# Borx25/CPU-Raytracing-experiments

Hardware: AMD Instinct MI355X
Metric: Mray/s (primary+bounce) (higher is better)
Workload: dtype f32; 1 GPU; cfg4: 4096x4096 px, S(100000) spheres + SAH BVH, MIS, Policy.max_bounces=9 (primary+8 bounces), 5 buckets, 64 accumulations/step; fixed image, tile rows split over the GPUs; image=4096x4096, spheres=100000, max_bounces=9, buckets=5, parallelism=single GPU, batches_in_flight=1, accumulations_per_batch=63, accumulations_per_batch_limit=63

## Files before the change

cpu-raytracing-experiments_amd/__init__.py:

```python
from __future__ import annotations

import ctypes as C
import os
import subprocess

import numpy as np

from . import distributed as distributed
from . import hdr as hdr
from . import scene as scene
from .scene import MATERIAL, NODE, SPHERE, Camera, Scene

_HERE = os.path.dirname(os.path.abspath(__file__))
CSRC = os.path.join(_HERE, "csrc")
LIB_PATH = os.path.join(CSRC, "libmirt.so")

MIRT_OK, MIRT_NOT_READY = 0, 1
MIRT_NOT_CONVERGED = 2
NOISE_BINS = 2048
AOV_DEPTH, AOV_NORMAL, AOV_ALBEDO = 0, 1, 2
AOV_PLANES = 7
KERNEL_CLASSES = ("raygen", "trace", "shade", "shadow", "resolve")


# ... 44 lines not shown

def load_library():
    global _lib
    if _lib is not None:
        return _lib
    if not os.path.exists(LIB_PATH):
        raise MirtError(f"{LIB_PATH} not built — run __graft_entry__.build() (hipcc --offload-arch=gfx950); there is no CPU fallback")
    lib = C.CDLL(LIB_PATH)
    P, u32, i32, f, vp = C.c_void_p, C.c_uint32, C.c_int, C.c_float, C.c_void_p
    sigs = {
        "mirt_create": [i32, C.POINTER(P)],
        "mirt_destroy": [P],
        "mirt_bvh_build": [vp, u32, vp, C.POINTER(u32), vp],
        "mirt_light_list": [vp, u32, vp, u32, vp, C.POINTER(u32)],
        "mirt_set_scene": [P, vp, vp, u32, vp, u32, vp, u32, vp, u32, vp, vp, u32, u32],
        "mirt_set_camera": [P, vp, vp, f, f, f, f],
        "mirt_set_lens": [P, f, f], "mirt_get_lens": [P, C.POINTER(f), C.POINTER(f)],
        "mirt_pick_focus": [P, u32, u32, C.POINTER(f), C.POINTER(f)],
        "mirt_set_policy": [P, C.POINTER(Policy)],
        "mirt_get_policy": [P, C.POINTER(Policy)],
        "mirt_set_gloss_decay": [P, vp, u32],
        "mirt_set_stream_order": [P, u32], "mirt_get_stream_order": [P, C.POINTER(u32)],
        "mirt_resize": [P, u32, u32],
        "mirt_set_tile_range": [P, u32, u32], "mirt_set_tile_rows": [P, u32, u32],
        "mirt_reset": [P],
        "mirt_accumulate": [P, u32],
        "mirt_accumulate_async": [P, u32],
        "mirt_synchronize": [P],
        "mirt_get_accumulations": [P, C.POINTER(u32)],
        "mirt_accumulator_floats": [P, C.POINTER(C.c_size_t)],
        "mirt_read_accumulator": [P, vp],
        "mirt_accumulator_device": [P, C.POINTER(vp), C.POINTER(C.c_size_t)],
        "mirt_load_accumulator": [P, vp, i32, u32],
        "mirt_render": [P, vp],
        "mirt_set_aov": [P, u32], "mirt_get_aov": [P, C.POINTER(u32)],
        "mirt_aov_floats": [P, C.POINTER(C.c_size_t)],
        "mirt_read_aov": [P, vp],
        "mirt_aov_device": [P, C.POINTER(vp), C.POINTER(C.c_size_t)],
        "mirt_load_aov": [P, vp, i32],
        "mirt_render_aov": [P, i32, vp],
        "mirt_noise": [P, f, vp, vp, vp, C.POINTER(NoiseStats)],
        "mirt_noise_quantile": [vp, C.c_double, C.POINTER(f)],
        "mirt_accumulate_until": [P, C.POINTER(StopRule), C.POINTER(NoiseStats), C.POINTER(u32)],
        "mirt_get_counters": [P, C.POINTER(Counters)],
        "mirt_get_kernel_times": [P, C.POINTER(KernelTimes), i32],
        "mirt_get_stream": [P, C.POINTER(vp)],
        "mirt_debug_raygen": [P, u32, vp, vp],
        "mirt_debug_trace_closest": [P, C.c_size_t, vp, vp, vp, vp],
        "mirt_debug_trace_shadow": [P, C.c_size_t, vp, vp, vp, vp],
        "mirt_debug_math": [P, i32, C.c_size_t, vp, vp],
        "mirt_debug_info": [P, vp],
        "mirt_debug_tree": [P, vp, C.c_size_t, vp],
        "mirt_debug_primary_lists": [P, vp],
        "mirt_debug_allow_half_boxes": [P, i32],
    }
    G = C.c_void_p
    sigs.update({
        "mirt_group_create": [vp, i32, C.POINTER(G)],
        "mirt_group_destroy": [G],
        "mirt_group_size": [G, C.POINTER(i32)],
        "mirt_group_member": [G, i32, C.POINTER(P)],
        "mirt_group_set_scene": [G, vp, vp, u32, vp, u32, vp, u32, vp, u32, vp, vp, u32, u32],
        "mirt_group_set_camera": [G, vp, vp, f, f, f, f],
        "mirt_group_set_lens": [G, f, f],
        "mirt_group_pick_focus": [G, u32, u32, C.POINTER(f), C.POINTER(f)],
        "mirt_group_set_policy": [G, C.POINTER(Policy)],
        "mirt_group_set_gloss_decay": [G, vp, u32],
        "mirt_group_set_stream_order": [G, u32],
        "mirt_group_resize": [G, u32, u32],
        "mirt_group_reset": [G],
        "mirt_group_accumulate": [G, u32],
        "mirt_group_accumulate_async": [G, u32],
        "mirt_group_synchronize": [G],
        "mirt_group_get_accumulations": [G, C.POINTER(u32)],
        "mirt_group_get_counters": [G, C.POINTER(Counters)],
        "mirt_group_gather": [G],
        "mirt_group_last_gather_ms": [G, C.POINTER(C.c_double)],
        "mirt_group_accumulator_floats": [G, C.POINTER(C.c_size_t)],
        "mirt_group_read_accumulator": [G, vp],
        "mirt_group_render": [G, vp],
        "mirt_group_set_aov": [G, u32],
        "mirt_group_aov_floats": [G, C.POINTER(C.c_size_t)],
        "mirt_group_read_aov": [G, vp],
        "mirt_group_render_aov": [G, i32, vp],
        "mirt_group_noise": [G, f, vp, vp, vp, C.POINTER(NoiseStats)],
        "mirt_group_accumulate_until": [G, C.POINTER(StopRule), C.POINTER(NoiseStats), C.POINTER(u32)],
        "mirt_group_rccl_selftest": [i32, C.c_size_t],
    })
    for name, argtypes in sigs.items():
        fn = getattr(lib, name)
        fn.argtypes = argtypes
        fn.restype = C.c_int
    lib.mirt_last_error.argtypes = [P]
    lib.mirt_last_error.restype = C.c_char_p
    lib.mirt_group_last_error.argtypes = [P]
    lib.mirt_group_last_error.restype = C.c_char_p
    lib._declared = tuple(sigs) + ("mirt_last_error", "mirt_group_last_error")
    _lib = lib
    return lib


def _ptr(a: np.ndarray):
    return a.ctypes.data_as(C.c_void_p)


def bvh_build(geometry: np.ndarray):
# ... 265 lines not shown
        ptr = C.c_void_p(src) if is_device else _ptr(np.ascontiguousarray(src, dtype=np.float32))
        self._check(self._lib.mirt_load_aov(self._ctx, ptr, int(is_device)))

    def render_aov(self, which: int, out: np.ndarray = None):
        img = _aov_image(self.height, self.width, which, out)
        rc = self._check(self._lib.mirt_render_aov(self._ctx, int(which), _ptr(img)))
        return img if rc == MIRT_OK else None

    noise_quantile = staticmethod(noise_quantile)

    def _local_tiles(self) -> int:
        n = C.c_size_t(0)
        self._check(self._lib.mirt_accumulator_floats(self._ctx, C.byref(n)))
        return n.value // (self.policy.buckets * 768)

    def noise(self, floor: float = 0.0, want_map: bool = False, map_out: np.ndarray = None):
        return _noise(self._lib.mirt_noise, self._check, self._ctx, self.height, self.width, self._local_tiles(), floor, want_map, map_out)

    def accumulate_until(self, target: float, quantile: float = 0.95, floor: float = 0.0, check_every: int = None, max_accumulations: int = 1000):
        return _accumulate_until(self._lib.mirt_accumulate_until, self._check, self._ctx, self.policy.buckets, target, quantile, floor, check_every, max_accumulations)

    def counters(self) -> dict:
        c = Counters()
        self._check(self._lib.mirt_get_counters(self._ctx, C.byref(c)))
        return c.as_dict()

    def kernel_times(self, reset: bool = True) -> dict:
        t = KernelTimes()
        self._check(self._lib.mirt_get_kernel_times(self._ctx, C.byref(t), int(reset)))
        return {k: {"ms": t.ms[i], "launches": int(t.launches[i])} for i, k in enumerate(KERNEL_CLASSES)}

    def debug_info(self) -> dict:
        out = (C.c_uint32 * 8)()
        self._check(self._lib.mirt_debug_info(self._ctx, out))
        keys = ("records", "lds_records", "lds_spheres", "depth", "half_boxes", "trace_lds_bytes", "trace_workgroups_per_cu", "cus")
        d = dict(zip(keys, [int(v) for v in out]))
        d["wide"] = (d["half_boxes"] >> 1) & 1
        d["half_boxes"] &= 1
        return d

    def debug_tree(self):
        info = (C.c_uint32 * 4)()
        self._check(self._lib.mirt_debug_tree(self._ctx, None, 0, info))
        n, rec_bytes = int(info[0]), int(info[1])
        words = np.zeros((n, rec_bytes // 4), dtype=np.uint32)
        self._check(self._lib.mirt_debug_tree(self._ctx, _ptr(words), words.nbytes, info))
        return words, dict(zip(("records", "record_bytes", "layout", "depth"), [int(v) for v in info]))

    def debug_primary_lists(self) -> list:
        out = (C.c_uint32 * 10)()
        self._check(self._lib.mirt_debug_primary_lists(self._ctx, out))
        return [int(v) for v in out]

    def stream_handle(self) -> int:
        p = C.c_void_p()
        self._check(self._lib.mirt_get_stream(self._ctx, C.byref(p)))
        return p.value

    def debug_raygen(self, accumulations: int):
        n = (self.width // 16) * (self.height // 16) * 256
        p = np.empty((3, n), dtype=np.float32)
        d = np.empty((3, n), dtype=np.float32)
        self._check(self._lib.mirt_debug_raygen(self._ctx, accumulations, _ptr(p), _ptr(d)))
        return p, d

    def debug_trace_closest(self, p: np.ndarray, d: np.ndarray):
        p = np.ascontiguousarray(p, dtype=np.float32); d = np.ascontiguousarray(d, dtype=np.float32)
        n = p.shape[1]
        tfar = np.empty(n, dtype=np.float32); prim = np.empty(n, dtype=np.int32)
        self._check(self._lib.mirt_debug_trace_closest(self._ctx, n, _ptr(p), _ptr(d), _ptr(tfar), _ptr(prim)))
        return tfar, prim

    def debug_trace_shadow(self, p: np.ndarray, d: np.ndarray, tfar: np.ndarray):
        p = np.ascontiguousarray(p, dtype=np.float32); d = np.ascontiguousarray(d, dtype=np.float32)
        tfar = np.ascontiguousarray(tfar, dtype=np.float32)
        n = p.shape[1]
        occ = np.empty(n, dtype=np.uint8)
        self._check(self._lib.mirt_debug_trace_shadow(self._ctx, n, _ptr(p), _ptr(d), _ptr(tfar), _ptr(occ)))
        return occ

    def debug_math(self, fn: int, inputs: np.ndarray, n_out: int) -> np.ndarray:
        inputs = np.ascontiguousarray(inputs, dtype=np.float32)
        n = inputs.shape[-1]
        out = np.empty((n_out, n), dtype=np.float32)
        self._check(self._lib.mirt_debug_math(self._ctx, fn, n, _ptr(inputs), _ptr(out)))
        return out


class GroupRenderer:

    def __init__(self, scene: Scene, devices=(0,), max_bounces: int = 16, buckets: int = 5, mis: bool = True, use_bvh: bool = True,
                 count_traffic: bool = False, max_batch: int = 0, streams: int = 0, reference_tree: bool = False, gpu_build: bool = False,
                 brdf: int = 0, gloss_decay=None, exact_stream_order: bool = False, aov: bool = False, lens: bool = False):
        self._lib = load_library()
        self._g = C.c_void_p()
        self._lens_follows_camera = bool(lens)
        dev = (C.c_int * len(devices))(*devices)
        rc = self._lib.mirt_group_create(dev, len(devices), C.byref(self._g))
        if rc != MIRT_OK:
            raise MirtError(f"mirt_group_create failed ({rc}): {self._lib.mirt_group_last_error(None).decode()}")
        self.scene, self.devices = scene, tuple(devices)
        self.width = self.height = 0
        self.framebuffer = None
        self.policy = Policy(max_bounces, buckets, int(mis), int(use_bvh), int(count_traffic), 0, max_batch, int(reference_tree), int(streams), int(gpu_build), 0,
                             int(brdf))
        self._check(self._lib.mirt_group_set_policy(self._g, C.byref(self.policy)))
# ... 159 lines not shown
```

cpu-raytracing-experiments_amd/csrc/kernels.hpp:

```cpp
#pragma once
#include <hip/hip_runtime.h>
#include <stdint.h>
#include "device_math.hpp"

namespace mirt {

constexpr uint32_t kBlock = 256;
constexpr uint32_t kShadeBlock = 512;
constexpr uint32_t kTraceBlock = 1024;
constexpr uint32_t kLdsStack = 16;
constexpr uint32_t kLdsStackWide = 12;
constexpr uint32_t kLeafBit = 0x80000000u;
constexpr uint32_t kTileSize = 256;
constexpr uint32_t kTileRoot = 16;
constexpr uint32_t kStack = 64;
constexpr uint32_t kDestAccum = 0x80000000u;

struct SceneDev {
	const float4* recs;
	const float4* spheres;
	const int32_t* prim_mat;
	const float4* light_sphere;
	const float4* light_emit;
	const float4* mat_albedo;
	const float4* mat_emission;
	const float4* hdri;
	uint32_t n_spheres, n_recs, n_mat, n_lights;
	uint32_t lds_recs;
	uint32_t lds_spheres;
	uint32_t half_boxes;
	uint32_t wide;
	uint32_t chunk_max;
	uint32_t leaf_batch;
	uint32_t refill_idle;
	uint32_t stack16;
	float ambient[3];
	int32_t hdri_w, hdri_h;
	float hdri_fw, hdri_fh;
	uint32_t has_ambient;
	uint32_t use_bvh;
};

struct StreamBuf {
	float *px, *py, *pz, *dx, *dy, *dz;
	float *tr, *tg, *tb;
	uint32_t* path;
};
struct ShadowBuf {
	float *px, *py, *pz;
	float *dx, *dy, *dz, *tfar;
	float *sr, *sg, *sb;
	float *er, *eg, *eb;
	uint32_t* dest;
};
struct FrameParams {
	CameraParams cam;
// ... 752 lines not shown
	};
	auto store_result = [&](uint32_t pix, const Trav& t, bool) {
		const bool over = static_cast<uint32_t>(t.prim) > kCandMax;
		cand[pix] = over ? kCandOverflow : static_cast<uint32_t>(t.prim);
		const unsigned long long m = __ballot(over);
		if (over) {
			const uint32_t leader = static_cast<uint32_t>(__ffsll(static_cast<long long>(m))) - 1u;
			uint32_t first = 0;
			if (lane_id() == leader) first = atomicAdd(ov_count, static_cast<uint32_t>(__popcll(m)));
			first = __builtin_amdgcn_readlane(first, leader);
			if (ov_pix) ov_pix[first + mask_rank(m)] = pix;
		}
	};
	trace_queue<kCollect, COUNT>(sc, tl, Queue{ nullptr, 0u }, n, work, unused, c_nodes, c_spheres, load_ray, store_result, Collect{ cand, rho, n });
	if (COUNT) { wave_sum(c_nodes, &ctr->nodes); wave_sum(c_spheres, &ctr->spheres); }
}
constexpr uint32_t kCandRegs = 3;
template <bool COUNT>
__global__ __launch_bounds__(kBlock) void k_primary_hits(SceneDev sc, FrameParams fp, const uint32_t* __restrict__ cand, HitRec* __restrict__ hit_out, DevCounters* ctr) {
	if (blockIdx.x == 0 && threadIdx.x == 0 && fp.n_pix) atomicAdd(&ctr->rays, static_cast<unsigned long long>(fp.n_pix) * fp.batch_n);
	uint32_t c_spheres = 0;
	const float ox = fp.cam.pos[0], oy = fp.cam.pos[1], oz = fp.cam.pos[2];
	for (uint32_t pix = blockIdx.x * kBlock + threadIdx.x; pix < fp.n_pix; pix += gridDim.x * kBlock) {
		const uint32_t cnt = cand[pix];
		if (cnt == kCandOverflow) continue;
		uint32_t tile; int32_t x, y;
		pixel_xy(fp, pix, tile, x, y);
		const uint32_t seed = (tile * kTileSize + (pix & 255u)) * (fp.max_bounces * 2u + 1u);
		float4 s[kCandRegs]; int32_t id[kCandRegs];
		for (uint32_t k = 0; k < kCandRegs; k++) {
			id[k] = k < cnt ? static_cast<int32_t>(cand[static_cast<size_t>(k + 1u) * fp.n_pix + pix]) : -1;
			s[k] = sc.spheres[id[k] < 0 ? 0 : id[k]];
		}
		for (uint32_t slot = 0; slot < fp.batch_n; slot++) {
			uint32_t rng = hash_2d(fp.acc_base + slot + 1u, seed);
			const float s0 = rand_unit_float(rng);
			const float s1 = rand_unit_float(rng);
			const f3 d = camera_ray_dir(fp.cam, x, y, s0, s1);
			float tfar = MIRT_FLT_MAX; int32_t prim = -1;
			for (uint32_t k = 0; k < kCandRegs; k++) if (id[k] >= 0) sphere_closest_tie(s[k], id[k], ox, oy, oz, d.x, d.y, d.z, tfar, prim);
			for (uint32_t k = kCandRegs; k < kCandMax; k++) {
				if (__ballot(k < cnt) == 0ull) break;
				if (k < cnt) {
					const uint32_t j = cand[static_cast<size_t>(k + 1u) * fp.n_pix + pix];
					sphere_closest_tie(sc.spheres[j], static_cast<int32_t>(j), ox, oy, oz, d.x, d.y, d.z, tfar, prim);
				}
			}
			if (COUNT) c_spheres += cnt;
			const size_t i = static_cast<size_t>(slot) * fp.n_pix + pix;
			hit_out[i] = HitRec{ tfar, prim };
		}
	}
	if (COUNT) wave_sum(c_spheres, &ctr->spheres);
}

constexpr uint32_t kAovPlanes = 7;
constexpr float kAovMissDepth = 1e4f;
template <bool LENS = false>
__global__ __launch_bounds__(kBlock) void k_first_hit_aov(SceneDev sc, FrameParams fp, const HitRec* __restrict__ hit_in, const float4* __restrict__ mat_colour, float* __restrict__ aov, LensParams lens) {
	f3 O{ fp.cam.pos[0], fp.cam.pos[1], fp.cam.pos[2] };
	for (uint32_t pix = blockIdx.x * kBlock + threadIdx.x; pix < fp.n_pix; pix += gridDim.x * kBlock) {
		uint32_t tile; int32_t x, y;
		pixel_xy(fp, pix, tile, x, y);
		const uint32_t seed = (tile * kTileSize + (pix & 255u)) * (fp.max_bounces * 2u + 1u);
		float* w = aov + static_cast<size_t>(pix >> 8) * (kAovPlanes * kTileSize) + (pix & 255u);
		float sum[kAovPlanes];
		for (uint32_t k = 0; k < kAovPlanes; k++) sum[k] = w[k * kTileSize];
		int32_t cached = -1;
		float4 hs = make_float4(0.0f, 0.0f, 0.0f, 0.0f), colour = hs;
		for (uint32_t slot = 0; slot < fp.batch_n; slot++) {
			uint32_t rng = hash_2d(fp.acc_base + slot + 1u, seed);
			const float s0 = rand_unit_float(rng);
			const float s1 = rand_unit_float(rng);
			f3 D = camera_ray_dir(fp.cam, x, y, s0, s1);
			if (LENS) lens_ray(fp.cam, lens, D, fp.acc_base + slot + 1u, seed, fp.max_bounces, O, D);
			const HitRec h = hit_in[static_cast<size_t>(slot) * fp.n_pix + pix];
			if (h.prim < 0) { sum[0] += kAovMissDepth; continue; }
			if (h.prim != cached) { hs = sc.spheres[h.prim]; colour = mat_colour[sc.prim_mat[h.prim]]; cached = h.prim; }
			const float depth = h.tfar;
			const f3 hit{ O.x + D.x * depth, O.y + D.y * depth, O.z + D.z * depth };
			f3 N = normalize3(f3{ hit.x - hs.x, hit.y - hs.y, hit.z - hs.z });
			if (dot3(N, D) >= 0.0f) N = f3{ -N.x, -N.y, -N.z };
			sum[0] += depth;
			sum[1] += N.x; sum[2] += N.y; sum[3] += N.z;
			sum[4] += colour.x; sum[5] += colour.y; sum[6] += colour.z;
		}
		for (uint32_t k = 0; k < kAovPlanes; k++) w[k * kTileSize] = sum[k];
	}
}
constexpr int kAovDepth = 0, kAovNormal = 1, kAovAlbedo = 2;
__global__ __launch_bounds__(kBlock) void k_resolve_aov(const float* __restrict__ aov, float* __restrict__ out, uint32_t n_pix, uint32_t first_tile, uint32_t run_tiles,
                                                        uint32_t stride_tiles, uint32_t h_tiles, uint32_t width, int which, float accumulations) {
	for (uint32_t pix = blockIdx.x * kBlock + threadIdx.x; pix < n_pix; pix += gridDim.x * kBlock) {
		const float* src = aov + static_cast<size_t>(pix >> 8) * (kAovPlanes * kTileSize) + (pix & 255u);
		const uint32_t tile = global_tile(first_tile, run_tiles, stride_tiles, pix >> 8), ID = pix & 255u;
		const uint32_t x = kTileRoot * (tile % h_tiles) + (ID & 15u);
		const uint32_t y = kTileRoot * (tile / h_tiles) + (ID >> 4);
		const size_t at = static_cast<size_t>(y) * width + x;
		if (which == kAovDepth) { out[at] = src[0] / accumulations; continue; }
		const uint32_t first = which == kAovNormal ? 1u : 4u;
		f3 v{ src[first * kTileSize], src[(first + 1u) * kTileSize], src[(first + 2u) * kTileSize] };
		if (which == kAovNormal) v = dot3(v, v) == 0.0f ? f3{ 0.0f, 0.0f, 0.0f } : normalize3(v);
		else v = { v.x / accumulations, v.y / accumulations, v.z / accumulations };
		out[at * 3u] = v.x; out[at * 3u + 1u] = v.y; out[at * 3u + 2u] = v.z;
	}
}
// ... 680 lines not shown
```

cpu-raytracing-experiments_amd/csrc/mirt_capi.hip:

```cpp
#include "../../include/mirt.h"
#include "kernels.hpp"
#include "bvh_layout.hpp"
#include "bvh_build.hpp"
#include "lbvh_build.hpp"
#include "noise_host.hpp"

#include <hip/hip_runtime.h>
#include <algorithm>
#include <cstdarg>
#include <cstdint>
#include <cstdio>
#include <cstdlib>
#include <cstring>
#include <string>
#include <vector>

using namespace mirt;

namespace {

thread_local std::string g_create_error;

struct DeviceBuffer {
	void* ptr = nullptr;
// ... 330 lines not shown
float bundle_half_angle(const mirt_ctx* c) { return (0.7072f / std::fabs(c->camera.z)) * 1.01f + 1e-4f; }

void update_lens_axes(mirt_ctx* c) {
	const f3 r = camera_axis(c->camera.orient, f3{ 1.0f, 0.0f, 0.0f }), u = camera_axis(c->camera.orient, f3{ 0.0f, 1.0f, 0.0f }), f = camera_axis(c->camera.orient, f3{ 0.0f, 0.0f, -1.0f });
	c->lens.right[0] = r.x; c->lens.right[1] = r.y; c->lens.right[2] = r.z;
	c->lens.up[0] = u.x; c->lens.up[1] = u.y; c->lens.up[2] = u.z;
	c->lens.fwd[0] = f.x; c->lens.fwd[1] = f.y; c->lens.fwd[2] = f.z;
}
bool lens_on(const mirt_ctx* c) { return c->lens.aperture > 0.0f; }

FrameParams frame_params(const mirt_ctx* c, uint32_t acc_base, uint32_t batch_n) {
	FrameParams fp{};
	fp.cam = c->camera;
	fp.h_tiles = c->h_tiles;
	fp.first_tile = c->first_tile;
	fp.run_tiles = c->run_tiles ? c->run_tiles : 1u;
	fp.stride_tiles = c->stride_tiles;
	fp.n_pix = c->n_tiles * kTileSize;
	fp.pix_bits = pix_bits_of(c); fp.pix_mask = (1u << fp.pix_bits) - 1u;
	fp.acc_base = acc_base;
	fp.batch_n = batch_n;
	fp.max_bounces = c->policy.max_bounces;
	fp.buckets = c->policy.buckets;
	fp.n_lights = c->scene.n_lights;
	fp.mis = (c->policy.mis && c->scene.n_lights > 0) ? 1u : 0u;
	fp.first_groups = 1;
	fp.inv_n_pix = fp.n_pix ? 1.0f / static_cast<float>(fp.n_pix) : 0.0f;
	fp.inv_h_tiles = fp.h_tiles ? 1.0f / static_cast<float>(fp.h_tiles) : 0.0f;
	fp.inv_run_tiles = 1.0f / static_cast<float>(fp.run_tiles);
	return fp;
}

SceneDev trace_scene(const mirt_ctx* c) {
	SceneDev sc = c->scene;
	sc.use_bvh = c->policy.use_bvh;
	sc.chunk_max = c->tune_chunk; sc.leaf_batch = c->tune_leaf_batch; sc.refill_idle = c->tune_refill_idle;
	return sc;
}

const decltype(&k_trace<true, kPrimaryNone>) kTrace[2][3] = {
	{ k_trace<true, kPrimaryNone>, k_trace<true, kPrimaryAll>, k_trace<true, kPrimaryList> },
	{ k_trace<false, kPrimaryNone>, k_trace<false, kPrimaryAll>, k_trace<false, kPrimaryList> } };
const decltype(&k_trace_fat<true, kPrimaryNone>) kTraceFat[2][3] = {
	{ k_trace_fat<true, kPrimaryNone>, k_trace_fat<true, kPrimaryAll>, k_trace_fat<true, kPrimaryList> },
	{ k_trace_fat<false, kPrimaryNone>, k_trace_fat<false, kPrimaryAll>, k_trace_fat<false, kPrimaryList> } };
const decltype(&k_primary_cand<true>) kPrimaryCand[2] = { k_primary_cand<true>, k_primary_cand<false> };
const decltype(&k_primary_hits<true>) kPrimaryHits[2] = { k_primary_hits<true>, k_primary_hits<false> };
const decltype(&k_shade<false, false>) kShade[2][2] = { { k_shade<false, false>, k_shade<false, true> }, { k_shade<true, false>, k_shade<true, true> } };
const decltype(&k_tile_stream<false>) kTileStream[2] = { k_tile_stream<false>, k_tile_stream<true> };
static_assert(kPrimaryNone == 0 && kPrimaryAll == 1 && kPrimaryList == 2, "kTrace / kTraceFat are indexed by PRIMARY");
const decltype(&k_trace<true, kPrimaryNone>) kTraceLens[2] = { k_trace<true, kPrimaryAll, true>, k_trace<false, kPrimaryAll, true> };
const decltype(&k_trace_fat<true, kPrimaryNone>) kTraceFatLens[2] = { k_trace_fat<true, kPrimaryAll, true>, k_trace_fat<false, kPrimaryAll, true> };
const decltype(&k_shade<false, false>) kShadeLens[2] = { k_shade<true, false, true>, k_shade<true, true, true> };

struct TraceLaunch {
	StreamBuf in; HitRec* hit;
	Queue closest_queue; uint32_t* closest_work;
	ShadowBuf sh; ShadowSink sink;
	Queue shadow_queue; uint32_t* shadow_work;
	FatList fat_closest, fat_shadow;
	const uint32_t* listed_pixels;
	DevCounters* ctr;
};
void launch_trace(const mirt_ctx* c, hipStream_t st, const SceneDev& sc, const FrameParams& fp, uint64_t n_rays, bool count, int primary, const TraceLaunch& t, bool lens = false) {
	hipLaunchKernelGGL(lens ? kTraceLens[!count] : kTrace[!count][primary], dim3(trace_grid(c, n_rays)), dim3(kTraceBlock), trace_lds(c), st, sc, fp, t.in, t.hit, t.closest_queue, t.closest_work,
	                   t.sh, t.sink, t.shadow_queue, t.shadow_work, t.fat_closest, t.fat_shadow, t.ctr, c->lens);
	const uint32_t fat_grid = sc.n_spheres > 4096 ? static_cast<uint32_t>(c->n_cu) * 2u : 64u;
	if (sc.use_bvh) hipLaunchKernelGGL(lens ? kTraceFatLens[!count] : kTraceFat[!count][primary], dim3(fat_grid), dim3(1024), 0, st, sc, fp, t.in, t.hit, t.fat_closest, t.sh, t.sink, t.fat_shadow, t.ctr, t.listed_pixels, c->lens);
}

int launch_tile_stream(mirt_ctx* c, hipStream_t st, const SceneDev& sc, const FrameParams& fp, uint32_t batch_n, float* contrib, DevCounters* ctr, bool count) {
	if (!c->gloss_decay_dev_valid) {
		HIP_TRY(c, sync_all(c));
		HIP_TRY(c, c->gloss_decay_dev.ensure(std::max<size_t>(c->gloss_decay.size(), 1) * sizeof(float)));
		if (!c->gloss_decay.empty()) HIP_TRY(c, hipMemcpy(c->gloss_decay_dev.ptr, c->gloss_decay.data(), c->gloss_decay.size() * sizeof(float), hipMemcpyHostToDevice));
		c->gloss_decay_dev_valid = true;
	}
	Bracket t(c, MIRT_K_TRACE, st);
	hipLaunchKernelGGL(kTileStream[c->policy.brdf != 0], dim3(c->n_tiles * batch_n), dim3(kTileSize), 0, st, sc, fp, contrib, ctr, c->mat_ggx.as<float4>(),
	                   c->gloss_decay_dev.as<float>(), static_cast<uint32_t>(c->gloss_decay.size()), count ? 1u : 0u);
	return MIRT_OK;
}

int build_primary_lists(mirt_ctx* c, const SceneDev& sc, const FrameParams& fp, bool count) {
	HIP_TRY(c, c->cand.ensure(static_cast<size_t>(fp.n_pix) * kCandStride * sizeof(uint32_t)));
	HIP_TRY(c, c->cand_listed.ensure(static_cast<size_t>(fp.n_pix) * sizeof(uint32_t)));
	HIP_TRY(c, c->cand_words.ensure(CandWords::kWords * sizeof(uint32_t)));
	if (!c->cand_built) HIP_TRY(c, hipEventCreateWithFlags(&c->cand_built, hipEventDisableTiming));
	const CandWords cw{ c->cand_words.as<uint32_t>() };
	HIP_TRY(c, hipMemsetAsync(cw.w, 0, CandWords::kWords * sizeof(uint32_t), c->stream));
	{ Bracket t(c, MIRT_K_TRACE);
	  const FatList none{ cw.unused_fat_count(), nullptr, 0u };
	  hipLaunchKernelGGL(kPrimaryCand[!count], dim3(trace_grid(c, fp.n_pix)), dim3(kTraceBlock), trace_lds(c), c->stream, sc, fp, c->cand.as<uint32_t>(), bundle_half_angle(c),
	                     cw.work(), none, c->counters.as<DevCounters>(), c->cand_listed.as<uint32_t>(), cw.listed_pixels()); }
	HIP_TRY(c, hipGetLastError());
	HIP_TRY(c, hipEventRecord(c->cand_built, c->stream));
	c->cand_gen++;
	c->cand_valid = true;
	return MIRT_OK;
}

int launch_first_hit_aov(mirt_ctx* c, PipeSlot& sl, hipStream_t st, const SceneDev& sc, const FrameParams& fp) {
	const bool pipelined = c->slots.size() > 1;
	if (pipelined) {
		if (!sl.aov_done) HIP_TRY(c, hipEventCreateWithFlags(&sl.aov_done, hipEventDisableTiming));
		if (c->aov_prev && c->aov_prev != sl.aov_done) HIP_TRY(c, hipStreamWaitEvent(st, c->aov_prev, 0));
// ... 1 lines not shown
	{ Bracket t(c, MIRT_K_RESOLVE, st);
	  const uint32_t grid = static_cast<uint32_t>(std::min<uint64_t>((static_cast<uint64_t>(fp.n_pix) + kBlock - 1) / kBlock, static_cast<uint64_t>(c->n_cu) * 64u));
	  hipLaunchKernelGGL(lens_on(c) ? k_first_hit_aov<true> : k_first_hit_aov<false>, dim3(grid), dim3(kBlock), 0, st, sc, fp, sl.hit, c->policy.brdf ? c->mat_ggx.as<float4>() : c->scene.mat_albedo,
	                     c->aov.as<float>(), c->lens); }
	if (pipelined) { HIP_TRY(c, hipEventRecord(sl.aov_done, st)); c->aov_prev = sl.aov_done; }
	return MIRT_OK;
}

int launch_batch(mirt_ctx* c, uint32_t batch_n) {
	FrameParams fp = frame_params(c, c->accumulations, batch_n);
	const uint32_t nb = c->policy.max_bounces;
	const uint64_t total = static_cast<uint64_t>(fp.n_pix) * batch_n;
	if (total == 0) { c->accumulations += batch_n; return MIRT_OK; }
	const bool pipelined = c->slots.size() > 1;
	PipeSlot& sl = c->slots[c->batch_seq % c->slots.size()];
	hipStream_t st = pipelined ? sl.stream : c->stream;
	const BatchCounters bc = batch_counters(c, sl);
	const float qn = c->camera.orient[0] * c->camera.orient[0] + c->camera.orient[1] * c->camera.orient[1] + c->camera.orient[2] * c->camera.orient[2] + c->camera.orient[3] * c->camera.orient[3];
	const bool lens = lens_on(c);
	const bool bundle = c->policy.use_bvh && c->scene.n_recs != 0 && !c->policy.trace_primary_rays && batch_n >= 3 && c->camera.z != 0.0f && std::fabs(qn - 1.0f) < 1e-4f && !c->stream_order && !lens;
	DevCounters* ctr = c->counters.as<DevCounters>();
	const float4* mat_ggx = c->mat_ggx.as<float4>();
	float* contrib = sl.contrib.as<float>();
	uint32_t* fat_lists = sl.fat.as<uint32_t>();
	const SceneDev sc = trace_scene(c);
	const bool count = c->policy.count_traffic != 0;
	const uint32_t sgrid = static_cast<uint32_t>(std::min<uint64_t>((total + kShadeBlock - 1) / kShadeBlock, static_cast<uint64_t>(c->n_cu) * c->tune_shade_wgs));
	{
		const uint64_t n_chunks = (static_cast<uint64_t>(fp.n_pix) + kShadeBlock - 1) / kShadeBlock;
		const uint64_t want = (8ull * sgrid + n_chunks - 1) / n_chunks;
		fp.first_groups = static_cast<uint32_t>(std::min<uint64_t>(std::max<uint64_t>(want, 1), batch_n));
	}

	if (pipelined && sl.in_use) HIP_TRY(c, hipStreamWaitEvent(st, sl.merged, 0));
	if (c->debug_poison_contrib)
		HIP_TRY(c, hipMemsetD32Async(reinterpret_cast<hipDeviceptr_t>(sl.contrib.ptr), 0x7fc0deadu, sl.contrib.bytes / sizeof(float), st));
	HIP_TRY(c, hipMemsetAsync(bc.w, 0, BatchCounters::words(nb) * sizeof(uint32_t), st));
	if (bundle) {
		if (!c->cand_valid || count) { const int r = build_primary_lists(c, sc, fp, count); if (r) return r; }
		if (pipelined && sl.cand_gen != c->cand_gen) { HIP_TRY(c, hipStreamWaitEvent(st, c->cand_built, 0)); sl.cand_gen = c->cand_gen; }
	}
	const CandWords cw{ c->cand_words.as<uint32_t>() };
	if (c->stream_order) {
		const int r = launch_tile_stream(c, st, sc, fp, batch_n, contrib, ctr, count);
		if (r) return r;
	} else {
		for (uint32_t bounce = 0; bounce < nb; bounce++) {
			const StreamBuf& in = sl.stream_buf[bounce & 1u];
			const StreamBuf& out = sl.stream_buf[(bounce & 1u) ^ 1u];
			const bool shadow_pending = fp.mis && bounce > 0;
			const bool lists = bounce == 0 && bundle;
			{ Bracket t(c, MIRT_K_TRACE, st);
			  if (lists) {
			    const uint32_t hgrid = static_cast<uint32_t>(std::min<uint64_t>((static_cast<uint64_t>(fp.n_pix) + kBlock - 1) / kBlock, static_cast<uint64_t>(c->n_cu) * 64u));
			    hipLaunchKernelGGL(kPrimaryHits[!count], dim3(hgrid), dim3(kBlock), 0, st, sc, fp, c->cand.as<uint32_t>(), sl.hit, ctr);
			  }
			  const ShadowSink sink{ in.path, in.px, in.py, in.pz, contrib, batch_n, fp.pix_bits, nullptr };
			  StreamBuf rays = in;
			  if (lists) rays.path = c->cand_listed.as<uint32_t>();
			  const TraceLaunch tl{ rays, sl.hit, lists ? Queue{ cw.listed_pixels(), 0u } : bc.stream_queue(bounce), bc.closest_work(bounce),
			                        sl.shadow_buf, sink, shadow_pending ? bc.shadow_queue(bounce - 1) : bc.empty_queue(), bc.shadow_work(shadow_pending ? bounce - 1 : 0),
			                        bc.fat_closest(bounce, fat_lists), bc.fat_shadow(bounce, fat_lists), lists ? cw.listed_pixels() : nullptr, ctr };
			  launch_trace(c, st, sc, fp, total, count, lists ? kPrimaryList : bounce == 0 ? kPrimaryAll : kPrimaryNone, tl, bounce == 0 && lens); }
			if (bounce == 0 && c->aov_on) { const int r = launch_first_hit_aov(c, sl, st, sc, fp); if (r) return r; }
			{ Bracket t(c, MIRT_K_SHADE, st);
			  const float decay = bounce < c->gloss_decay.size() ? c->gloss_decay[bounce] : 0.0f;
			  hipLaunchKernelGGL(bounce == 0 && lens ? kShadeLens[c->policy.brdf != 0] : kShade[bounce == 0][c->policy.brdf != 0], dim3(sgrid), dim3(kShadeBlock), 0, st, sc, fp, in, sl.hit, out, sl.shadow_buf, bounce,
			                     bc.stream_queue(bounce), bc.stream_queue(bounce + 1), bc.shadow_queue(bounce), contrib, ctr, mat_ggx, decay, c->lens); }
		}
	}
	HIP_TRY(c, hipGetLastError());
	if (pipelined) {
		HIP_TRY(c, hipEventRecord(sl.batch_done, st));
		HIP_TRY(c, hipStreamWaitEvent(c->stream, sl.batch_done, 0));
	}
	{ Bracket t(c, MIRT_K_RESOLVE);
	  hipLaunchKernelGGL(k_merge_contrib, dim3(grid_for(c, static_cast<uint64_t>(c->n_tiles) * (kTileSize / 4u))), dim3(kBlock), 0, c->stream,
	                     c->accumulator.as<float4>(), sl.contrib.as<float4>(), c->n_tiles, c->policy.buckets, batch_n, fp.acc_base); }
	HIP_TRY(c, hipGetLastError());
	if (pipelined) { HIP_TRY(c, hipEventRecord(sl.merged, c->stream)); sl.in_use = true; }
	c->batch_seq++;
	c->accumulations += batch_n;
	if (c->policy.profile && c->pending.size() > 512) harvest(c);
	return MIRT_OK;
}

template <class T>
int upload(mirt_ctx* c, DeviceBuffer& buf, const std::vector<T>& host) {
	HIP_TRY(c, buf.ensure(std::max<size_t>(host.size(), 1) * sizeof(T)));
	if (!host.empty()) HIP_TRY(c, hipMemcpyAsync(buf.ptr, host.data(), host.size() * sizeof(T), hipMemcpyHostToDevice, c->stream));
	return MIRT_OK;
}

int check_ready(mirt_ctx* c) {
	if (!c) return MIRT_ERR_ARG;
	if (!c->have_scene) return fail(c, MIRT_ERR_STATE, "mirt_set_scene has not been called");
	if (!c->have_camera) return fail(c, MIRT_ERR_STATE, "mirt_set_camera has not been called");
	if (c->width == 0 && c->height == 0) return fail(c, MIRT_ERR_STATE, "mirt_resize has not been called");
	return MIRT_OK;
}

int flush_deferred(mirt_ctx* c) {
	if (!c->deferred) return MIRT_OK;
	const uint32_t n = c->deferred;
	c->deferred = 0;
	HIP_TRY(c, hipSetDevice(c->device));
	int r = ensure_streams(c); if (r) return r;
	return launch_batch(c, n);
// ... 699 lines not shown
	if (!c) return MIRT_ERR_ARG;
	if (!c->have_scene) return fail(c, MIRT_ERR_STATE, "mirt_set_scene has not been called");
	if (!p_xyz || !dir_xyz || !tfar_out || !prim_out || n == 0 || n >= (1ull << 31)) return fail(c, MIRT_ERR_ARG, "bad arguments");
	std::vector<HitRec> hits(n);
	const int r = debug_trace(c, "debug_trace_closest", n, p_xyz, dir_xyz, nullptr, hits.data());
	if (r == MIRT_OK) for (size_t i = 0; i < n; i++) { tfar_out[i] = hits[i].tfar; prim_out[i] = hits[i].prim; }
	return r;
}

int mirt_debug_trace_shadow(mirt_ctx* c, size_t n, const float* p_xyz, const float* dir_xyz, const float* tfar, uint8_t* occluded_out) {
	if (!c) return MIRT_ERR_ARG;
	if (!c->have_scene) return fail(c, MIRT_ERR_STATE, "mirt_set_scene has not been called");
	if (!p_xyz || !dir_xyz || !tfar || !occluded_out || n == 0 || n >= (1ull << 31)) return fail(c, MIRT_ERR_ARG, "bad arguments");
	std::vector<uint32_t> occ(n);
	const int r = debug_trace(c, "debug_trace_shadow", n, p_xyz, dir_xyz, tfar, occ.data());
	if (r == MIRT_OK) for (size_t i = 0; i < n; i++) occluded_out[i] = occ[i] ? 1 : 0;
	return r;
}

int mirt_debug_math(mirt_ctx* c, int fn, size_t n, const float* in, float* out) {
	if (!c) return MIRT_ERR_ARG;
	static const int n_in[11] = { 1, 2, 1, 2, 2, 6, 8, 3, 10, 9, 1 }, n_out[11] = { 2, 1, 1, 3, 3, 10, 5, 5, 3, 6, 1 };
	if (fn < 0 || fn > 10 || !in || !out || n == 0 || n >= (1u << 28)) return fail(c, MIRT_ERR_ARG, "bad arguments");
	HIP_TRY(c, hipSetDevice(c->device));
	ScopedBuffer din, dout;
	HIP_TRY(c, din.ensure(n * n_in[fn] * 4)); HIP_TRY(c, dout.ensure(n * n_out[fn] * 4));
	HIP_TRY(c, hipMemcpy(din.ptr, in, n * n_in[fn] * 4, hipMemcpyHostToDevice));
	hipLaunchKernelGGL(k_debug_math, dim3(grid_for(c, n)), dim3(kBlock), 0, c->stream, fn, static_cast<uint32_t>(n), din.as<float>(), dout.as<float>());
	hipError_t e = hipGetLastError();
	if (e == hipSuccess) e = hipStreamSynchronize(c->stream);
	if (e == hipSuccess) e = hipMemcpy(out, dout.ptr, n * n_out[fn] * 4, hipMemcpyDeviceToHost);
	if (e != hipSuccess) return fail(c, MIRT_ERR_HIP, "debug_math: %s", hipGetErrorString(e));
	return MIRT_OK;
}

int mirt_debug_primary_lists(mirt_ctx* c, uint32_t hist[10]) {
	int r = check_ready(c); if (r) return r;
	if (!hist) return fail(c, MIRT_ERR_ARG, "hist is NULL");
	if (!c->policy.use_bvh || c->scene.n_recs == 0 || c->n_tiles == 0) return fail(c, MIRT_ERR_STATE, "needs policy.use_bvh, a tree and at least one tile");
	{ const int fr = flush_deferred(c); if (fr) return fr; }
	HIP_TRY(c, hipSetDevice(c->device));
	if ((r = ensure_streams(c))) return r;
	HIP_TRY(c, sync_all(c));
	const FrameParams fp = frame_params(c, 0, 1);
	if (!c->cand_valid && (r = build_primary_lists(c, trace_scene(c), fp, false))) return r;
	std::vector<uint32_t> host(static_cast<size_t>(fp.n_pix));
	HIP_TRY(c, hipMemcpyAsync(host.data(), c->cand.ptr, host.size() * 4, hipMemcpyDeviceToHost, c->stream));
	HIP_TRY(c, hipStreamSynchronize(c->stream));
	for (int k = 0; k < 10; k++) hist[k] = 0;
	for (size_t p = 0; p < fp.n_pix; p++) { const uint32_t n = host[p]; hist[n == kCandOverflow ? 9 : std::min<uint32_t>(n, 8u)]++; }
	return MIRT_OK;
}

int mirt_debug_info(mirt_ctx* c, uint32_t out[8]) {
	if (!c || !out) return MIRT_ERR_ARG;
	const SceneDev& s = c->scene;
	const LdsPlan p = lds_plan(c);
	out[0] = s.n_recs; out[1] = s.lds_recs; out[2] = s.lds_spheres; out[3] = c->bvh_depth; out[4] = s.half_boxes | (s.wide << 1);
	out[5] = p.launch_bytes; out[6] = p.wgs_per_cu; out[7] = static_cast<uint32_t>(c->n_cu);
	return MIRT_OK;
}
int mirt_debug_tree(mirt_ctx* c, void* dst, size_t capacity_bytes, uint32_t info[4]) {
	if (!c) return MIRT_ERR_ARG;
	if (!info) return fail(c, MIRT_ERR_ARG, "debug_tree: info is NULL");
	if (!c->have_scene) return fail(c, MIRT_ERR_STATE, "mirt_set_scene has not been called");
	const SceneDev& s = c->scene;
	const uint32_t rec_bytes = (s.half_boxes && !s.wide) ? 32u : 64u;
	info[0] = s.n_recs; info[1] = rec_bytes; info[2] = s.wide ? 2u : s.half_boxes ? 1u : 0u; info[3] = c->bvh_depth;
	if (!dst) return MIRT_OK;
	const size_t bytes = static_cast<size_t>(s.n_recs) * rec_bytes;
	if (capacity_bytes < bytes) return fail(c, MIRT_ERR_ARG, "debug_tree: %zu bytes of capacity, the records take %zu", capacity_bytes, bytes);
	if (bytes == 0) return MIRT_OK;
	HIP_TRY(c, hipSetDevice(c->device));
	HIP_TRY(c, hipStreamSynchronize(c->stream));
	HIP_TRY(c, hipMemcpy(dst, s.recs, bytes, hipMemcpyDeviceToHost));
	return MIRT_OK;
}
int mirt_debug_allow_half_boxes(mirt_ctx* c, int allow) { if (!c) return MIRT_ERR_ARG; c->allow_half = allow != 0; return MIRT_OK; }

}
```

include/mirt.h:

```cpp
#ifndef MIRT_H
#define MIRT_H

#include <stddef.h>
#include <stdint.h>

#ifdef __cplusplus
extern "C" {
#endif

#define MIRT_OK              0
#define MIRT_NOT_READY       1
#define MIRT_ERR_ARG        -1
#define MIRT_ERR_HIP        -2
#define MIRT_ERR_STATE      -3
#define MIRT_ERR_NO_DEVICE  -4

#define MIRT_TILE_ROOT     16u
#define MIRT_TILE_SIZE    256u
#define MIRT_MAX_MATERIALS 63u
#define MIRT_MAX_BUCKETS   16u
#define MIRT_BVH_STACK     64u

typedef struct mirt_sphere {
	float   position[3];
// ... 129 lines not shown
	uint32_t max_accumulations;
} mirt_stop_rule;
int mirt_accumulate_until(mirt_ctx* ctx, const mirt_stop_rule* rule, mirt_noise_stats* last, uint32_t* issued);

int mirt_get_counters(mirt_ctx* ctx, mirt_counters* out);
int mirt_get_kernel_times(mirt_ctx* ctx, mirt_kernel_times* out, int reset);
int mirt_get_stream(mirt_ctx* ctx, void** hip_stream);

typedef struct mirt_group mirt_group;
int mirt_group_create(const int* devices, int n, mirt_group** out);
int mirt_group_destroy(mirt_group* group);
const char* mirt_group_last_error(const mirt_group* group);
int mirt_group_size(const mirt_group* group, int* n);
int mirt_group_member(mirt_group* group, int index, mirt_ctx** ctx);
int mirt_group_set_scene(mirt_group* group,
                         const mirt_sphere* geometry, const mirt_sphere* bvh_prims, uint32_t n_spheres,
                         const mirt_bvh_node* nodes, uint32_t n_nodes,
                         const mirt_material* materials, uint32_t n_materials,
                         const int32_t* lights, uint32_t n_lights,
                         const float ambient_color[3], const float* hdri_rgba, uint32_t hdri_w, uint32_t hdri_h);
int mirt_group_set_camera(mirt_group* group, const float pos[3], const float orient_xyzw[4], float half_width, float half_height, float z, float exposure);
int mirt_group_set_lens(mirt_group* group, float aperture_radius, float focus_depth);
int mirt_group_pick_focus(mirt_group* group, uint32_t x, uint32_t y, float* distance, float* depth);
int mirt_group_set_policy(mirt_group* group, const mirt_policy* policy);
int mirt_group_set_gloss_decay(mirt_group* group, const float* decay, uint32_t n);
int mirt_group_set_stream_order(mirt_group* group, uint32_t exact);
int mirt_group_resize(mirt_group* group, uint32_t width, uint32_t height);
int mirt_group_reset(mirt_group* group);
int mirt_group_accumulate(mirt_group* group, uint32_t n_calls);
int mirt_group_accumulate_async(mirt_group* group, uint32_t n_calls);
int mirt_group_synchronize(mirt_group* group);
int mirt_group_get_accumulations(const mirt_group* group, uint32_t* accumulations);
int mirt_group_get_counters(mirt_group* group, mirt_counters* out);
int mirt_group_gather(mirt_group* group);
int mirt_group_last_gather_ms(const mirt_group* group, double* ms);
int mirt_group_accumulator_floats(const mirt_group* group, size_t* n_floats);
int mirt_group_read_accumulator(mirt_group* group, float* host_dst);
int mirt_group_render(mirt_group* group, float* rgba_host);
int mirt_group_set_aov(mirt_group* group, uint32_t on);
int mirt_group_aov_floats(const mirt_group* group, size_t* n_floats);
int mirt_group_read_aov(mirt_group* group, float* host_dst);
int mirt_group_render_aov(mirt_group* group, int which, float* out);
int mirt_group_noise(mirt_group* group, float floor, float* map_out, float* tile_out, uint32_t* hist_out, mirt_noise_stats* stats);
int mirt_group_accumulate_until(mirt_group* group, const mirt_stop_rule* rule, mirt_noise_stats* last, uint32_t* issued);
int mirt_group_rccl_selftest(int device, size_t n_floats);

int mirt_debug_raygen(mirt_ctx* ctx, uint32_t accumulations, float* p_xyz, float* dir_xyz);
int mirt_debug_trace_closest(mirt_ctx* ctx, size_t n, const float* p_xyz, const float* dir_xyz, float* tfar_out, int32_t* primID_out);
int mirt_debug_trace_shadow(mirt_ctx* ctx, size_t n, const float* p_xyz, const float* dir_xyz, const float* tfar, uint8_t* occluded_out);
int mirt_debug_math(mirt_ctx* ctx, int fn, size_t n, const float* in, float* out);
int mirt_debug_info(mirt_ctx* ctx, uint32_t out[8]);
int mirt_debug_tree(mirt_ctx* ctx, void* dst, size_t capacity_bytes, uint32_t info[4]);
int mirt_debug_primary_lists(mirt_ctx* ctx, uint32_t hist[10]);
int mirt_debug_allow_half_boxes(mirt_ctx* ctx, int allow);

#ifdef __cplusplus
}
#endif
#endif
```

Baseline: 9481 Mray/s.

## Add wave-per-pixel-run primary hit kernel with lane-per-sample mapping

Adds a primary-hit kernel in which each wavefront handles a run of 16 pixels in a tile row and each lane handles one accumulation sample. Candidate sphere IDs and sphere data are loaded once per pixel and broadcast across lanes with readlane, and the loads for the next pixels are prefetched. Results pass through LDS and are transposed so the global writes stay coalesced. The aim is to remove redundant per-sample candidate and sphere loads and the divergence of the per-pixel kernel, at the cost of LDS staging, wave barriers, and idle lanes when a group holds fewer than 64 samples. The new path is used only when the batch has at least 32 accumulations. A debug API for reading candidate counts is also added.

```diff
diff --git a/cpu-raytracing-experiments_amd/__init__.py b/cpu-raytracing-experiments_amd/__init__.py
--- a/cpu-raytracing-experiments_amd/__init__.py
+++ b/cpu-raytracing-experiments_amd/__init__.py
@@ -120,6 +120,7 @@
         "mirt_debug_info": [P, vp],
         "mirt_debug_tree": [P, vp, C.c_size_t, vp],
         "mirt_debug_primary_lists": [P, vp],
+        "mirt_debug_primary_counts": [P, vp, C.c_size_t],
         "mirt_debug_allow_half_boxes": [P, i32],
     }
     G = C.c_void_p
@@ -491,6 +492,13 @@
         self._check(self._lib.mirt_debug_primary_lists(self._ctx, out))
         return [int(v) for v in out]
 
+    def debug_primary_counts(self) -> np.ndarray:
+        n = C.c_size_t(0)
+        self._check(self._lib.mirt_accumulator_floats(self._ctx, C.byref(n)))
+        out = np.zeros((n.value // (self.policy.buckets * 768), 256), dtype=np.uint32)
+        self._check(self._lib.mirt_debug_primary_counts(self._ctx, _ptr(out), out.size))
+        return out
+
     def stream_handle(self) -> int:
         p = C.c_void_p()
         self._check(self._lib.mirt_get_stream(self._ctx, C.byref(p)))
diff --git a/cpu-raytracing-experiments_amd/csrc/hits_wave_map.hpp b/cpu-raytracing-experiments_amd/csrc/hits_wave_map.hpp
--- /dev/null
+++ b/cpu-raytracing-experiments_amd/csrc/hits_wave_map.hpp
@@ -0,0 +1,17 @@
+#pragma once
+#include <stdint.h>
+
+namespace mirt {
+
+constexpr uint32_t kWaveHitsMinBatch = 32;
+constexpr uint32_t kWaveHitsRun = 16;
+constexpr uint32_t kWaveHitsPasses = kWaveHitsRun;
+constexpr uint32_t kWaveHitsStage = kWaveHitsRun * 64u;
+
+constexpr uint32_t hits_wave_groups(uint32_t batch_n) { return (batch_n + 63u) >> 6; }
+constexpr uint32_t hits_wave_group_slots(uint32_t batch_n, uint32_t g) { return batch_n - g * 64u < 64u ? batch_n - g * 64u : 64u; }
+constexpr uint32_t hits_wave_stage_index(uint32_t p, uint32_t s) { return p * 64u + (s ^ p); }
+constexpr uint32_t hits_wave_out_pixel(uint32_t lane) { return lane & (kWaveHitsRun - 1u); }
+constexpr uint32_t hits_wave_out_slot(uint32_t lane, uint32_t pass) { return pass * (64u / kWaveHitsRun) + lane / kWaveHitsRun; }
+
+}
diff --git a/cpu-raytracing-experiments_amd/csrc/kernels.hpp b/cpu-raytracing-experiments_amd/csrc/kernels.hpp
--- a/cpu-raytracing-experiments_amd/csrc/kernels.hpp
+++ b/cpu-raytracing-experiments_amd/csrc/kernels.hpp
@@ -2,6 +2,7 @@
 #include <hip/hip_runtime.h>
 #include <stdint.h>
 #include "device_math.hpp"
+#include "hits_wave_map.hpp"
 
 namespace mirt {
 
@@ -860,6 +861,69 @@
 		}
 	}
 	if (COUNT) wave_sum(c_spheres, &ctr->spheres);
+}
+constexpr uint32_t kWaveHitsWaves = kBlock / 64u;
+static_assert(kCandMax < 64u && kTileSize % kWaveHitsRun == 0u && kWaveHitsRun == kTileRoot, "lane k holds list entry k; a run is one row of a tile");
+template <bool COUNT>
+__global__ __launch_bounds__(kBlock) void k_primary_hits_wave(SceneDev sc, FrameParams fp, const uint32_t* __restrict__ cand, HitRec* __restrict__ hit_out, DevCounters* ctr) {
+	__shared__ HitRec stage[kWaveHitsWaves][kWaveHitsStage];
+	const uint32_t lane = lane_id();
+	const uint32_t wave = static_cast<uint32_t>(__builtin_amdgcn_readfirstlane(static_cast<int>(threadIdx.x >> 6)));
+	const uint32_t n_runs = fp.n_pix / kWaveHitsRun, n_groups = hits_wave_groups(fp.batch_n);
+	const uint32_t out_p = hits_wave_out_pixel(lane);
+	uint32_t c_spheres = 0;
+	const float ox = fp.cam.pos[0], oy = fp.cam.pos[1], oz = fp.cam.pos[2];
+	for (uint32_t run = blockIdx.x * kWaveHitsWaves + wave; run < n_runs; run += gridDim.x * kWaveHitsWaves) {
+		const uint32_t base = static_cast<uint32_t>(__builtin_amdgcn_readfirstlane(static_cast<int>(run * kWaveHitsRun)));
+		const uint32_t cnt_v = cand[base + out_p];
+		const uint32_t skip = static_cast<uint32_t>(__ballot(cnt_v == kCandOverflow)) & 0xffffu;
+		if (skip == 0xffffu) continue;
+		uint32_t tile; int32_t x0, y;
+		pixel_xy(fp, base, tile, x0, y);
+		const uint32_t seed0 = tile * kTileSize + (base & 255u), seed_mul = fp.max_bounces * 2u + 1u;
+		auto count_of = [&](uint32_t p) { return static_cast<uint32_t>(__builtin_amdgcn_readlane(static_cast<int>(cnt_v), static_cast<int>(p))) + 1u; };
+		auto load_ids = [&](uint32_t p) { const uint32_t c1 = count_of(p); return cand[static_cast<size_t>(min(lane + 1u, c1 ? c1 - 1u : 0u)) * fp.n_pix + base + p]; };
+		auto load_sphere = [&](uint32_t p, uint32_t j) { return sc.spheres[lane + 1u < count_of(p) ? j : 0u]; };
+		for (uint32_t g = 0; g < n_groups; g++) {
+			const uint32_t slot = g * 64u + lane;
+			uint32_t id_cur = load_ids(0), id_next = load_ids(1);
+			float4 s_cur = load_sphere(0, id_cur);
+			for (uint32_t p = 0; p < kWaveHitsRun; p++) {
+				const float4 s_next = load_sphere(min(p + 1u, kWaveHitsRun - 1u), id_next);
+				const uint32_t id_next2 = load_ids(min(p + 2u, kWaveHitsRun - 1u));
+				const uint32_t cnt1 = count_of(p);
+				if (cnt1 != 0u) {
+					const uint32_t cnt = cnt1 - 1u;
+					uint32_t rng = hash_2d(fp.acc_base + slot + 1u, (seed0 + p) * seed_mul);
+					const float s0 = rand_unit_float(rng);
+					const float s1 = rand_unit_float(rng);
+					const f3 d = camera_ray_dir(fp.cam, x0 + static_cast<int32_t>(p), y, s0, s1);
+					float tfar = MIRT_FLT_MAX; int32_t prim = -1;
+					for (uint32_t k = 0; k < cnt; k++) {
+						const int32_t j = __builtin_amdgcn_readlane(static_cast<int>(id_cur), static_cast<int>(k));
+						const float4 s{ __int_as_float(__builtin_amdgcn_readlane(__float_as_int(s_cur.x), static_cast<int>(k))), __int_as_float(__builtin_amdgcn_readlane(__float_as_int(s_cur.y), static_cast<int>(k))),
+						                __int_as_float(__builtin_amdgcn_readlane(__float_as_int(s_cur.z), static_cast<int>(k))), __int_as_float(__builtin_amdgcn_readlane(__float_as_int(s_cur.w), static_cast<int>(k))) };
+						sphere_closest_tie(s, j, ox, oy, oz, d.x, d.y, d.z, tfar, prim);
+					}
+					if (COUNT && slot < fp.batch_n) c_spheres += cnt;
+					stage[wave][hits_wave_stage_index(p, lane)] = HitRec{ tfar, prim };
+				}
+				id_cur = id_next; id_next = id_next2; s_cur = s_next;
+			}
+			__builtin_amdgcn_fence(__ATOMIC_RELEASE, "wavefront"); __builtin_amdgcn_wave_barrier(); __builtin_amdgcn_fence(__ATOMIC_ACQUIRE, "wavefront");
+			const uint32_t n_slots = hits_wave_group_slots(fp.batch_n, g);
+			if (!((skip >> out_p) & 1u)) {
+				for (uint32_t pass = 0; pass < kWaveHitsPasses; pass++) {
+					const uint32_t s = hits_wave_out_slot(lane, pass);
+					if (s >= n_slots) break;
+					hit_out[static_cast<size_t>(g * 64u + s) * fp.n_pix + base + out_p] = stage[wave][hits_wave_stage_index(out_p, s)];
+				}
+			}
+			__builtin_amdgcn_fence(__ATOMIC_RELEASE, "wavefront"); __builtin_amdgcn_wave_barrier(); __builtin_amdgcn_fence(__ATOMIC_ACQUIRE, "wavefront");
+		}
+	}
+	if (COUNT) wave_sum(c_spheres, &ctr->spheres);
+	if (blockIdx.x == 0 && threadIdx.x == 0 && fp.n_pix) atomicAdd(&ctr->rays, static_cast<unsigned long long>(fp.n_pix) * fp.batch_n);
 }
 
 constexpr uint32_t kAovPlanes = 7;
diff --git a/cpu-raytracing-experiments_amd/csrc/mirt_capi.hip b/cpu-raytracing-experiments_amd/csrc/mirt_capi.hip
--- a/cpu-raytracing-experiments_amd/csrc/mirt_capi.hip
+++ b/cpu-raytracing-experiments_amd/csrc/mirt_capi.hip
@@ -406,6 +406,7 @@
 const decltype(&k_trace<true, kPrimaryNone>) kTraceLens[2] = { k_trace<true, kPrimaryAll, true>, k_trace<false, kPrimaryAll, true> };
 const decltype(&k_trace_fat<true, kPrimaryNone>) kTraceFatLens[2] = { k_trace_fat<true, kPrimaryAll, true>, k_trace_fat<false, kPrimaryAll, true> };
 const decltype(&k_shade<false, false>) kShadeLens[2] = { k_shade<true, false, true>, k_shade<true, true, true> };
+const decltype(&k_primary_hits_wave<true>) kPrimaryHitsWave[2] = { k_primary_hits_wave<true>, k_primary_hits_wave<false> };
 
 struct TraceLaunch {
 	StreamBuf in; HitRec* hit;
@@ -513,8 +514,14 @@
 			const bool lists = bounce == 0 && bundle;
 			{ Bracket t(c, MIRT_K_TRACE, st);
 			  if (lists) {
-			    const uint32_t hgrid = static_cast<uint32_t>(std::min<uint64_t>((static_cast<uint64_t>(fp.n_pix) + kBlock - 1) / kBlock, static_cast<uint64_t>(c->n_cu) * 64u));
-			    hipLaunchKernelGGL(kPrimaryHits[!count], dim3(hgrid), dim3(kBlock), 0, st, sc, fp, c->cand.as<uint32_t>(), sl.hit, ctr);
+			    if (batch_n >= kWaveHitsMinBatch) {
+			      const uint64_t runs = static_cast<uint64_t>(fp.n_pix) / kWaveHitsRun;
+			      const uint32_t wgrid = static_cast<uint32_t>(std::min<uint64_t>((runs + kWaveHitsWaves - 1) / kWaveHitsWaves, static_cast<uint64_t>(c->n_cu) * 20u));
+			      hipLaunchKernelGGL(kPrimaryHitsWave[!count], dim3(wgrid), dim3(kBlock), 0, st, sc, fp, c->cand.as<uint32_t>(), sl.hit, ctr);
+			    } else {
+			      const uint32_t hgrid = static_cast<uint32_t>(std::min<uint64_t>((static_cast<uint64_t>(fp.n_pix) + kBlock - 1) / kBlock, static_cast<uint64_t>(c->n_cu) * 64u));
+			      hipLaunchKernelGGL(kPrimaryHits[!count], dim3(hgrid), dim3(kBlock), 0, st, sc, fp, c->cand.as<uint32_t>(), sl.hit, ctr);
+			    }
 			  }
 			  const ShadowSink sink{ in.path, in.px, in.py, in.pz, contrib, batch_n, fp.pix_bits, nullptr };
 			  StreamBuf rays = in;
@@ -1320,6 +1327,22 @@
 	return MIRT_OK;
 }
 
+int mirt_debug_primary_counts(mirt_ctx* c, uint32_t* counts, size_t capacity) {
+	int r = check_ready(c); if (r) return r;
+	if (!counts) return fail(c, MIRT_ERR_ARG, "counts is NULL");
+	if (!c->policy.use_bvh || c->scene.n_recs == 0 || c->n_tiles == 0) return fail(c, MIRT_ERR_STATE, "needs policy.use_bvh, a tree and at least one tile");
+	{ const int fr = flush_deferred(c); if (fr) return fr; }
+	HIP_TRY(c, hipSetDevice(c->device));
+	if ((r = ensure_streams(c))) return r;
+	HIP_TRY(c, sync_all(c));
+	const FrameParams fp = frame_params(c, 0, 1);
+	if (capacity < fp.n_pix) return fail(c, MIRT_ERR_ARG, "debug_primary_counts: room for %zu counts, %u local pixels", capacity, fp.n_pix);
+	if (!c->cand_valid && (r = build_primary_lists(c, trace_scene(c), fp, false))) return r;
+	HIP_TRY(c, hipMemcpyAsync(counts, c->cand.ptr, static_cast<size_t>(fp.n_pix) * 4, hipMemcpyDeviceToHost, c->stream));
+	HIP_TRY(c, hipStreamSynchronize(c->stream));
+	return MIRT_OK;
+}
+
 int mirt_debug_info(mirt_ctx* c, uint32_t out[8]) {
 	if (!c || !out) return MIRT_ERR_ARG;
 	const SceneDev& s = c->scene;
diff --git a/include/mirt.h b/include/mirt.h
--- a/include/mirt.h
+++ b/include/mirt.h
@@ -205,6 +205,7 @@
 int mirt_debug_info(mirt_ctx* ctx, uint32_t out[8]);
 int mirt_debug_tree(mirt_ctx* ctx, void* dst, size_t capacity_bytes, uint32_t info[4]);
 int mirt_debug_primary_lists(mirt_ctx* ctx, uint32_t hist[10]);
+int mirt_debug_primary_counts(mirt_ctx* ctx, uint32_t* counts, size_t capacity);
 int mirt_debug_allow_half_boxes(mirt_ctx* ctx, int allow);
 
 #ifdef __cplusplus
```

New measurement: 9594 Mray/s, median of 6. +1.2%, better.
